# exosports/BART

Hardware: AMD Instinct MI355X
Metric: forward spectra/sec (100 layers x 1e4 wavenumbers) (higher is better)
Workload: dtype f64; 1 GPU; H2O+CO+CO2+CH4 eclipse, 100 layers x 10000 wavenumbers, 10 walkers batched per GPU per step (BASELINE config 3), opacity-table path, 27 T planes, H2-H2 CIA, 5 ray angles, toomuch 10, SURVEY 8d opacities, every step its own profile preparation; nlayers=100, nwave=10000, integ=1, cut=slant, cia_interp=spline, kappa_model=survey8d, parallelism=single GPU

## Files before the change

### bart_amd/build.py

```python
from __future__ import annotations

import os
import subprocess
import sys
from concurrent.futures import ThreadPoolExecutor

HERE = os.path.dirname(os.path.abspath(__file__))
CSRC = os.path.join(HERE, "csrc")
LIB = os.path.join(HERE, "libbartrt.so")
CLI = os.path.join(HERE, "transit")
SOURCES = ["rt_eclipse_angles.hip", "rt_eclipse_slant_ilp.hip", "rt_eclipse_qadj.hip", "rt_eclipse_i0.hip", "rt_eclipse_i1.hip", "rt_eclipse_i2.hip", "rt_eclipse_i0_ilp.hip", "rt_eclipse_i1_ilp.hip", "lbl.hip",
           "transit_geom.hip", "contrib.hip",
           "kernels.hip", "capi.hip", "engine.hip", "step.hip", "comm.hip", "mcmc.hip", "share.hip", "svc.hip", "rtc.hip", "io.cpp"]
HEADERS = ["engine.hpp", "kernels.hpp", "rt_eclipse.hpp", "rt_eclipse_s1.hpp", "rt_eclipse_s1s.hpp", "rt_eclipse_qadj.hpp", "kernel_table.inc", "imw_tab.hpp", "integ.hpp", "step.hpp", "lbl.hpp", "voigt_coef.hpp", "expint_coef.hpp", "prep.hpp", "io.hpp", "share.hpp", "svc.hpp", "svc_core.hpp", "rtc.hpp", "contrib.hpp", "comm.hpp", "devbuf.hpp",
           "transit_main.cpp", "../../include/bartrt.h"]


ILP = ["-mllvm", "-amdgpu-sched-strategy=max-ilp"]
EXTRA_FLAGS = {"rt_eclipse_i0_ilp.hip": ILP, "rt_eclipse_i1_ilp.hip": ILP, "rt_eclipse_slant_ilp.hip": ILP}
ANGLE_SIZES = tuple(int(x) for x in os.environ.get("BARTRT_AOT_ANGLES", "").split())
VARIANTS = {"rt_eclipse_angles.hip": [("rt_eclipse_a%d" % n, ["-DBARTRT_ANGLES=%d" % n, *ILP]) for n in ANGLE_SIZES]}
ANGLE_FLAG = "-DBARTRT_ANGLE_SIZES(X)=" + " ".join("X(%d)" % n for n in ANGLE_SIZES)

RT_OBJECT_PREFIXES = ("rt_eclipse_", "kernels", "engine")
BUILD_ID_INC = os.path.join(CSRC, "build_id.inc")


def _elf_section(blob: bytes, want: str):
    import struct
    if blob[:4] != b"\x7fELF" or blob[4] != 2:
        return None
    shoff, = struct.unpack_from("<Q", blob, 0x28)
    shentsize, shnum, shstrndx = struct.unpack_from("<HHH", blob, 0x3A)
    if shnum == 0:
# ... 146 lines not shown
```

### bart_amd/csrc/capi.hip

```cpp
#include <cstring>
#include <stdexcept>
#include <string>

#include "../../include/bartrt.h"
#include "comm.hpp"
#include "contrib.hpp"
#include "engine.hpp"
#include "lbl.hpp"
#include "share.hpp"
#include "step.hpp"
#include "rtc.hpp"
#include "svc.hpp"

#include <climits>
#include <cstdio>
#include <cstdlib>

#include <sys/stat.h>
#include <unistd.h>

using namespace bartrt;

static Engine *g_eng = nullptr;
static ChainService *g_svc = nullptr;
// ... 637 lines not shown
    if (ncolumns) *ncolumns = nc;
    if (wn_per_column) *wn_per_column = e->walked_info.wn_per_column;
    if (kernel && kernel_len > 0) {
      std::snprintf(kernel, (size_t)kernel_len, "%s%s%s%s", e->walked_info.kernel, e->walked_info.rtc ? " [instantiated at run time]" : "",
                    e->walked_info.prep_folded ? " [prepares its own walkers]" : "",
                    e->walked_info.window ? " [table through a moving window]" : "");
    }
    if (walked && n > 0) {
      if ((size_t)cap < (size_t)n * nc) throw std::invalid_argument("walked_end: buffer too small");
      HIPCHK(hipMemcpy(walked, e->d_walked, sizeof(int) * (size_t)n * nc, hipMemcpyDeviceToHost));
    }
    return BARTRT_OK;
  });
}

int bartrt_get_rtc_stats(int *available, int *compiled, int *from_disk, int *failed, double *compile_seconds) {
  const RtcStats st = rtc_stats();
  if (available) *available = rtc_available() ? 1 : 0;
  if (compiled) *compiled = st.compiled;
  if (from_disk) *from_disk = st.from_disk;
  if (failed) *failed = st.failed;
  if (compile_seconds) *compile_seconds = st.compile_seconds;
  return BARTRT_OK;
}

int bartrt_rtc_compile(const char *expr, int ilp, long *code_bytes) {
  if (!expr) return fail(BARTRT_EINVAL, "rtc_compile: null expression");
  std::string why;
  const long n = rtc_compile_only(expr, ilp != 0, why);
  if (code_bytes) *code_bytes = n;
// ... 278 lines not shown
```

### bart_amd/csrc/engine.hip

```cpp
#include "engine.hpp"
#include "lbl.hpp"
#include "contrib.hpp"
#include "share.hpp"
#include "step.hpp"
#include "svc.hpp"

#include <algorithm>
#include <climits>
#include <cmath>
#include <cstdlib>
#include <cstring>

#include <sys/stat.h>
#include <unistd.h>

namespace bartrt {

EngineStream::~EngineStream() {
  for (auto e : ev) (void)hipEventDestroy(e);
  if (stream) (void)hipStreamDestroy(stream);
}

Engine::~Engine() {
  delete step;
// ... 628 lines not shown
  pa.cloud_rup = cloud_rup; pa.cloud_rdown = cloud_rdown; pa.cloud_ext = cloud_ext;
  pa.coef = records.coef; pa.idx = records.idx; pa.kstop = records.kstop;
  pa.ok = d_okp ? d_okp : rec[0].ok.get();
  pa.rad_out = d_rad;
  pa.over = prep_over_once;
  pa.rtop = solution == 1 ? d_rtop.get() : nullptr;
  pa.ds = solution == 1 ? d_ds.get() : nullptr;
  return pa;
}

static int rt_block() {
  static const int b = [] { const char *e = std::getenv("BARTRT_BLOCK"); return e ? std::atoi(e) : 64; }();
  return (b == 128 || b == 256) ? b : 64;
}

RtArgs Engine::rt_args(const PrepArgs &pa, const Prefetch &pf, double *d_spec_out, bool want_tau, const double *d_ext,
                       bool lbl_fused, bool over_cloud, bool timed, hipStream_t st) {
  const int n = pa.nwalkers, block = rt_block();
  RtArgs r = rt;
  r.nwalkers = n;
  r.nsel = sel_walkers > n ? sel_walkers : 0;
  if (kernel_by_local) r.Wfull = r.W;
  r.coef = pa.coef; r.idx = pa.idx; r.kstop = pa.kstop;
  r.ext = d_ext;
  r.nprep = 0;
  if (pf.want_next) {
    const RecordSet &next = rec[1 - pf.bset];
    PrepArgs pn = pa;
    pn.nwalkers = pf_req_n;
    pn.prof = pf_req_prof;
// ... 15 lines not shown
  r.intens_out = nullptr;
  if (want_intens && n == 1 && solution == 0) {
    d_intens.reserve((size_t)A * W());
    r.intens_out = d_intens;
  }
  r.ntiles = (r.W + block - 1) / block;
  r.rtop = d_rtop; r.ds = d_ds;
  r.slog = nullptr;
  if (cut_slant && integ == 1 && solution == 0 && !lbl_fused) {
    const size_t need = slant_log_bytes(n, r.ntiles, block, A);
    if (need > d_slog.count()) {
      HIPCHK(hipDeviceSynchronize());
      d_slog.reserve(need);
    }
    r.slog = d_slog.get();
  }
  r.inv_starrad2 = solution == 1 ? 1.0 / (starrad * starrad) : 0.0;
  r.transparent = transparent ? 1 : 0;
  r.ev_start = r.ev_stop = nullptr;
  if (timed) {
    while ((int)ev.size() < ev_used + 2) {
      hipEvent_t e;
      HIPCHK(hipEventCreate(&e));
      ev.push_back(e);
    }
    if (lbl_fused) HIPCHK(hipEventRecord(ev[ev_used], st));
    else { r.ev_start = ev[ev_used]; r.ev_stop = ev[ev_used + 1]; }
  }
  r.walked_out = nullptr;
  if (want_walked && solution == 0 && !lbl_fused) {
// ... 61 lines not shown
```

### bart_amd/csrc/engine.hpp

```cpp
#pragma once
#include <hip/hip_runtime.h>

#include <string>
#include <vector>

#include "devbuf.hpp"
#include "io.hpp"
#include "kernels.hpp"

namespace bartrt {

hipError_t launch_prep(const PrepArgs &a, hipStream_t st);
hipError_t launch_rt(const RtArgs &a, int block, hipStream_t st, RtLaunchInfo *info = nullptr);
hipError_t launch_rt_folded(const RtArgs &a, const PrepArgs &prep, int block, hipStream_t st, RtLaunchInfo *info, bool *folded);
hipError_t launch_transit(const RtArgs &a, hipStream_t st, RtLaunchInfo *info = nullptr);
hipError_t launch_chord_table(const PrepArgs &a, hipStream_t st);
hipError_t launch_grid_transpose(const double *src, double *dst, long planes, int M, int W, hipStream_t st);

int parse_integ(const std::string &v);
int resolve_share_mode(const TCfg &cfg, bool no_service);

struct TableShare;
struct StepArgs;
struct Lbl;
// ... 83 lines not shown
  const double *pf_have_prof = nullptr;
  int pf_have_n = 0, pf_have_buf = 0;
  struct PrepSettings {
    double refradius, gsurf, cloudtop, scat_value, cloud_rup, cloud_rdown, cloud_ext;
    int has_cloud, scat_flag;
    bool operator==(const PrepSettings &o) const {
      return refradius == o.refradius && gsurf == o.gsurf && cloudtop == o.cloudtop && scat_value == o.scat_value &&
             cloud_rup == o.cloud_rup && cloud_rdown == o.cloud_rdown && cloud_ext == o.cloud_ext &&
             has_cloud == o.has_cloud && scat_flag == o.scat_flag;
    }
  };
  hipStream_t pf_have_stream = nullptr;
  PrepSettings pf_have_set{};
  int cap2 = 0;
  DevBuf<char> d_slog;
  StepArgs *step = nullptr;
  Lbl *lbl = nullptr;
  CfState *cf = nullptr;

  ~Engine();
  void init(int argc, const char **argv);
  void setup(const TCfg &cfg_in, int shard_rank, int shard_n);
  void read_settings();
  void generate_missing_opacity_file(int shard_rank);
  void read_atmosphere();
  void read_grid(OpacityHeader &oh, int shard_rank, int shard_n);
  void read_geometry();
  void open_device();
  void upload_table(const OpacityHeader &oh);
  void resample_cia(std::vector<double> &cia_planes, std::vector<double> &cia_temp);
// ... 24 lines not shown
```

### bart_amd/csrc/kernels.hip

```cpp
#include "integ.hpp"
#include "kernels.hpp"
#include "prep.hpp"

#include <cmath>
#include <cstdio>
#include <cstdlib>
#include <cstring>
#include <utility>

namespace bartrt {

template <int INTEG>
bool launch_rt_spec(const RtArgs &a, int block, hipStream_t st, KernelMode mode, bool force_window,
                    bool allow_sq, hipError_t &err, RtLaunchInfo *info, const PrepArgs *fold = nullptr);
extern template bool launch_rt_spec<0>(const RtArgs &, int, hipStream_t, KernelMode, bool, bool, hipError_t &, RtLaunchInfo *, const PrepArgs *);
extern template bool launch_rt_spec<1>(const RtArgs &, int, hipStream_t, KernelMode, bool, bool, hipError_t &, RtLaunchInfo *, const PrepArgs *);
extern template bool launch_rt_spec<2>(const RtArgs &, int, hipStream_t, KernelMode, bool, bool, hipError_t &, RtLaunchInfo *, const PrepArgs *);

__global__ __launch_bounds__(256) void prep_profiles(PrepArgs p) {
  extern __shared__ double sm[];
  prep_block(p, blockIdx.x, sm);
}

__device__ inline void block_to_work_g(int b, int nwalkers, int &tile, int &walker) {
// ... 169 lines not shown
    if (e != hipSuccess) return e;
    allowed = sh;
  }
  BARTRT_RT_LAUNCH((rt_eclipse<AT, -1, -1, INTEG>), dim3(nblocks), dim3(block), sh, st, a);
  return hipGetLastError();
}

KernelMode rt_kernel_mode() {
  static const KernelMode mode = [] {
    const char *e = std::getenv("BARTRT_KERNEL");
    if (!e || !*e) return KernelMode::kDefault;
    static const std::pair<const char *, KernelMode> names[] = {
        {"generic", KernelMode::kGeneric}, {"mono", KernelMode::kMono}, {"mono_occ", KernelMode::kMonoOcc},
        {"mono_ilp", KernelMode::kMonoIlp}, {"split", KernelMode::kSplit}, {"quad", KernelMode::kQuad},
        {"octo", KernelMode::kOcto}, {"hexa", KernelMode::kHexa}, {"r32", KernelMode::kR32},
        {"adj8", KernelMode::kAdj8}, {"adj16", KernelMode::kAdj16}};
    for (const auto &n : names)
      if (std::strcmp(e, n.first) == 0) return n.second;
    std::fprintf(stderr, "libbartrt: BARTRT_KERNEL=%s is not a kernel form (generic, mono, mono_occ, mono_ilp, split, quad, "
                         "octo, hexa, r32, adj8, adj16); ignored\n", e);
    return KernelMode::kDefault;
  }();
  return mode;
}
static bool rt_force_window() {
  static const bool v = std::getenv("BARTRT_WINDOW") != nullptr;
  return v;
}
static bool rt_allow_sq() {
  static const bool v = [] {
    const char *e = std::getenv("BARTRT_SQ");
    return !(e && e[0] == '0');
  }();
  return v;
}
// ... 43 lines not shown
```

### bart_amd/csrc/kernels.hpp

```cpp
#pragma once
#ifndef __HIPCC_RTC__
#include <hip/hip_runtime.h>
#include <hip/hip_ext.h>
#include <cstdint>
#else
typedef struct ihipEvent_t *hipEvent_t;
namespace std {
template <class T, T v> struct integral_constant { static constexpr T value = v; using value_type = T; constexpr operator T() const { return v; } };
using true_type = integral_constant<bool, true>;
using false_type = integral_constant<bool, false>;
template <bool B, class T, class F> struct conditional { using type = T; };
template <class T, class F> struct conditional<false, T, F> { using type = F; };
template <bool B, class T, class F> using conditional_t = typename conditional<B, T, F>::type;
}
#endif

#define BARTRT_MC_LIST(X) \
  X(1, 0) X(1, 1) X(1, 2) X(2, 0) X(2, 1) X(2, 2) X(3, 0) X(3, 1) X(3, 2) X(4, 0) X(4, 1) X(4, 2) \
  X(5, 0) X(5, 1) X(5, 2) X(6, 0) X(6, 1) X(6, 2)                                                 \
  X(1, 4) X(2, 4) X(3, 4) X(4, 4) X(5, 4) X(6, 4)
#define BARTRT_QADJ_LIST(X) BARTRT_MC_LIST(X)
#define BARTRT_EXT_C_LIST(X) X(0) X(1) X(2) X(4)

#define BARTRT_RT_LAUNCH(kernel, grid, block, sh, st, args) \
// ... 102 lines not shown
  int ref_ib;
  double ref_f;
  double ref_lnp;
  double gsurf, refradius;
  int scat_flag, iH2, iHe, has_cloud;
  double scat_value, cloudtop;
  double cloud_rup, cloud_rdown, cloud_ext;
  const double *over;
  double *coef;
  idx_t *idx;
  int *kstop;
  unsigned char *ok;
  double *rad_out;
  double *rtop;
  double *ds;
};

struct RtArgs {
  int L, M, Nt, C, A, W, nwalkers, ntiles;
  int nsel;
  int Wfull;
  const double *kappa;
  const double *cia;
  unsigned long long kappa_bytes, cia_bytes;
  int window;
  const double *ext;
  const double *wn;
  const double *coef;
  const idx_t *idx;
  const int *kstop;
// ... 2 lines not shown
  int cut_slant;
  double toomuch;
  double invmu[kMaxAngles];
  double wgt[kMaxAngles];
  double wq[kMaxAngles];
  double mu[kMaxAngles];
  double thr[kMaxAngles];
  double thrb[kMaxAngles];
  int drank[kMaxAngles];
  void *slog;
  double *spec;
  double *tau_out;
  int *last_out;
  double *intens_out;
  int *walked_out;
  const double *rtop, *ds;
  double inv_starrad2;
  int transparent;
  hipEvent_t ev_start, ev_stop;
  int nprep;
  PrepArgs prep_next;
};
__host__ __device__ inline int prep_slots(int nprep) { return (nprep + 7) / 8 * 8; }

inline void slant_thresholds(RtArgs &r) {
  for (int a = 0; a < r.A; a++) {
    const double im = r.invmu[a];
    double t = r.toomuch / im;
    if (!(t == t) || t > 1.7e308 || t < 0.0) { r.thr[a] = t < 0.0 ? -1.0 : 1.7976931348623157e308; continue; }
    for (int it = 0; it < 64 && t * im > r.toomuch; it++) t = __builtin_nextafter(t, 0.0);
// ... 15 lines not shown
inline size_t slant_log_bytes(int nwalkers, int ntiles, int block, int A) {
  return (size_t)nwalkers * (size_t)ntiles * (size_t)block * (size_t)A * 20u;
}

struct RtLaunchInfo {
  const char *kernel = "";
  int wn_per_column = 64;
  int ncolumns = 0;
  bool prep_fused = false;
  bool prep_folded = false;
  bool rtc = false;
  bool window = false;
};

#ifndef __HIPCC_RTC__
enum class KernelMode { kDefault, kGeneric, kMono, kMonoOcc, kMonoIlp, kSplit, kQuad, kOcto, kHexa, kR32, kAdj8, kAdj16 };
KernelMode rt_kernel_mode();
#endif

constexpr double kExpShift = 6755399441055744.0;
constexpr double kExpMin = -708.0;

__device__ __forceinline__ double exp_scale(double p, double shifted) {
  const int hi = __double2hiint(p) + (__double2loint(shifted) << 20);
  return __hiloint2double(hi, __double2loint(p));
}

__device__ __forceinline__ double exp_core(double x) {
  const double t = fma(x, 1.4426950408889634074, kExpShift);
  const double n = t - kExpShift;
  double r = fma(n, -6.93147180369123816490e-01, x);
// ... 146 lines not shown
```

### bart_amd/csrc/rt_eclipse.hpp

```cpp
#pragma once
#include "integ.hpp"
#include "kernels.hpp"
#include "prep.hpp"

#ifndef __HIPCC_RTC__
#include <cmath>
#include <cstdlib>
#include <type_traits>
#include <utility>
#endif

#ifndef BARTRT_WPE
#define BARTRT_WPE 4
#endif

namespace bartrt {

constexpr long kQuadMaxColumns = 640, kQuadMaxColumnsSimpson = 480;
constexpr long kQuadRaysMaxColumns = 80;
constexpr long kOctoRaysMaxColumns = 40;
constexpr int kFoldMaxWorkgroups = 512;
constexpr long kOctoMaxColumns = 400;
constexpr long kSplitMinColumns = 1025, kSplitMaxColumns = 1300;
constexpr long kIlpMaxColumns = 20000;
// ... 653 lines not shown
      };
      swap_angles(0, i);
      if (j == 0) j = i;
      swap_angles(r.A - 1, j);
      return true;
    }
  return false;
}

bool launch_rt_fast_ilp(const RtArgs &b, bool sq, int block, int nblocks, size_t sh, hipStream_t st, hipError_t &err);
bool launch_rt_fast_ext(const RtArgs &b, bool sq, int block, int nblocks, size_t sh, hipStream_t st, hipError_t &err);

bool launch_rt_slant(const RtArgs &b, int integ, bool sq, int block, int nblocks, size_t sh, hipStream_t st, hipError_t &err);
bool launch_rt_slant_ext(const RtArgs &b, int integ, bool sq, int block, int nblocks, size_t sh, hipStream_t st, hipError_t &err);
bool launch_rt_slant_out(const RtArgs &b, int block, int nblocks, size_t sh, hipStream_t st, hipError_t &err);

bool launch_rt_qadj(const RtArgs &b, bool sq, int rows, int nblocks, size_t sh, hipStream_t st, hipError_t &err);

#ifndef BARTRT_ANGLE_SIZES
#define BARTRT_ANGLE_SIZES(X)
#endif
#define BARTRT_DECL_ANGLES(N) \
  bool launch_rt_angles_##N(const RtArgs &b, int integ, int block, int nblocks, size_t sh, hipStream_t st, hipError_t &err);
BARTRT_ANGLE_SIZES(BARTRT_DECL_ANGLES)
#undef BARTRT_DECL_ANGLES

struct SpecLaunch {
  const RtArgs &a;
  RtArgs b;
  bool sq = false;
// ... 146 lines not shown
  static_assert(INTEG != kIntegSimpson, "the one-ray-per-lane form: rules 0 / 2");
  const LpGeom g = lp_geom(c, rows, 64 / rows / 5);
  const RtArgs &b = g.b;
  return (dispatch_mc(b.M, b.C, false, [&](auto m, auto cc, auto) {
            constexpr int M = decltype(m)::value, C = decltype(cc)::value;
            c.run(rows == 8 ? rt_eclipse_quad<5, M, C, false, 8, INTEG, true> : rt_eclipse_quad<5, M, C, false, 4, INTEG, true>,
                  g.nwg, 256, g.lds, b);
          }) ||
          rtc_try(c.info, false, dim3(g.nwg), dim3(256), g.lds, c.st, b, c.err, "rt_eclipse_quad<5, %d, %d, false, %d, %d, true>",
                  b.M, b.C, rows, INTEG)) &&
         c.launched(rows == 8 ? "rt_eclipse_quad<R=8, one ray per lane>" : "rt_eclipse_quad<R=4, one ray per lane>", g.wn, g.ncolumns,
                    false, b.window != 0);
}

template <int INTEG>
bool launch_form_slant(const SpecLaunch &c) {
  const RtArgs &b = c.b;
  const int nwg = c.workgroups(b.ntiles);
  const size_t lds = c.sh + c.shp;
  return (launch_rt_slant(b, INTEG, c.sq, c.block, nwg, lds, c.st, c.err) ||
          (rtc_single_wave_ok(b) &&
           (INTEG == kIntegSimpson
                ? rtc_try(c.info, true, dim3(nwg), dim3(c.block), lds, c.st, b, c.err, "rt_eclipse_simpson_slant<5, %d, %d, %s, %d>",
                          b.M, b.C, tf(c.sq), slant_sched(b.M, b.C, 1))
                : rtc_try(c.info, true, dim3(nwg), dim3(c.block), lds, c.st, b, c.err, "rt_eclipse_fast<5, %d, %d, %s, %d, 1, false, true>",
                          b.M, b.C, tf(c.sq), INTEG)))) &&
         c.launched(INTEG == kIntegSimpson ? "rt_eclipse_simpson_slant (ILP-scheduled build)" : "rt_eclipse_fast<SLANT> (ILP-scheduled build)",
                    c.block, b.ntiles);
}

template <int INTEG>
bool launch_form_quad(const SpecLaunch &c, int rows) {
  const LpGeom g = lp_geom(c, rows, 64 / rows);
  const RtArgs &b = g.b;
// ... 92 lines not shown
        const LpGeom g = lp_geom(c, adj_rows, 64 / adj_rows);
        if (fold && !g.folds) return false;
        if (launch_form_qadj(c, g, adj_rows)) return true;
      }
      const bool lp_forced = mode == KernelMode::kQuad || mode == KernelMode::kOcto || mode == KernelMode::kHexa ||
                             mode == KernelMode::kR32 || mode == KernelMode::kAdj8 || mode == KernelMode::kAdj16;
      if ((lp_forced || (dflt && other != kVarSingle)) && c.addressable(rows)) {
        const LpGeom g = lp_geom(c, rows, 64 / rows);
        if (fold && !g.folds) return false;
        if (launch_form_quad_allr<INTEG>(c, g, rows)) return true;
      }
      if (fold) return false;
    } else if ((mode == KernelMode::kQuad || mode == KernelMode::kOcto || (dflt && columns <= kQuadRaysMaxColumns)) && fits32) {
      if (launch_form_quad_rays<INTEG>(c, mode == KernelMode::kOcto || (dflt && columns <= kOctoRaysMaxColumns) ? 8 : 4)) return true;
    }
    return launch_form_slant<INTEG>(c);
  }
  constexpr long quad_max = INTEG == kIntegSimpson ? kQuadMaxColumnsSimpson : kQuadMaxColumns;
  if ((mode == KernelMode::kQuad || mode == KernelMode::kOcto || (dflt && columns <= quad_max)) && fits32 &&
      launch_form_quad<INTEG>(c, octo ? 8 : 4))
    return true;
  if constexpr (INTEG != kIntegSimpson) {
    if ((mode == KernelMode::kSplit || (dflt && columns >= kSplitMinColumns && columns <= kSplitMaxColumns)) &&
        launch_form_split<INTEG>(c))
      return true;
  }
  return launch_form_single<INTEG>(c, mode != KernelMode::kMonoOcc && (mode == KernelMode::kMonoIlp || columns < kIlpMaxColumns));
}

#endif
}
// ... 1 lines not shown
```

### bart_amd/csrc/rt_eclipse_s1s.hpp

```cpp
#pragma once
#include "integ.hpp"
#include "kernels.hpp"
#include "rt_eclipse_s1.hpp"

#ifndef __HIPCC_RTC__
#include <type_traits>
#endif

namespace bartrt {

#ifndef BARTRT_FLAG_CLAMP
#define BARTRT_FLAG_CLAMP 1
#endif
template <int A>
__device__ __forceinline__ double alive_flags(const RtArgs &p, double tm, double (&m)[A]) {
  double n = 0.0;
#if BARTRT_FLAG_CLAMP
  const double tb = tm * -4.149515568880993e180;
#pragma unroll
  for (int a = 0; a < A; a++) {
    asm("v_add_f64 %0, %1, %2 clamp" : "=v"(m[a]) : "v"(tb), "s"(p.thrb[a]));
    n += m[a];
  }
#else
#pragma unroll
  for (int a = 0; a < A; a++) {
    m[a] = tm <= p.thr[a] ? 1.0 : 0.0;
    n += m[a];
  }
#endif
  return n;
}

template <int AT, int MT, int CT, bool SQ, int SCHED = 1, bool EXT = false, bool OUT = false>
__global__ __launch_bounds__(256) __attribute__((amdgpu_waves_per_eu(OUT ? 1 : 2, BARTRT_WPE)))
void rt_eclipse_simpson_slant(RtArgs p) {
  extern __shared__ double smem[];
  constexpr int A = AT, M = MT, C = CT;
  constexpr int NC = 4 + 2 * M + 2 * C, NI = 1 + C, NLD = 2 * M + 2 * C;
  constexpr int NR = NLD + (EXT ? 1 : 0) > 0 ? NLD + (EXT ? 1 : 0) : 1;
  constexpr int AE = SQ ? A - 1 : A;
  constexpr int kBlk = 6;
  static_assert(kBlk - 2 <= kSimpsonPad, "the radius table's overrun entries");
  const int L = p.L, W = p.W;
  int bid = blockIdx.x;
  if (p.nprep > 0) {
    if (bid < p.nprep) { prep_block(p.prep_next, bid, smem); return; }
    bid -= prep_slots(p.nprep);
    if (bid < 0) return;
  }
  int tile, w;
  block_to_work(bid, p.nwalkers, tile, w);
  if (tile >= p.ntiles) return;

  double *sC = smem;
  idx_t *sI = reinterpret_cast<idx_t *>(smem + (size_t)L * NC);
  double *sWw = smem + (size_t)L * NC + (size_t)L * NI;
  const double *sW = sWw;
  stage2_to_lds(sC, p.coef + (size_t)w * L * NC, L * NC, sI, p.idx + (size_t)w * L * NI, L * NI, threadIdx.x,
                blockDim.x);
  const int kraw = p.kstop[w], kend = kstop_layer(kraw);
  const bool deck_on = kstop_deck(kraw);
  __syncthreads();
  simpson_radius_table(sWw, sC, NC, L, kend, threadIdx.x, blockDim.x);
  __syncthreads();

  const int i = tile * blockDim.x + threadIdx.x;
  const bool valid = i < W;
  const unsigned ii = valid ? (unsigned)i : (unsigned)(W - 1);
  const double nu = p.wn[ii];
  const double bnum = 2.0 * kH * nu * nu * nu * kLS * kLS;
  const double nu4 = (nu * nu) * (nu * nu);
  const TableLoader<M, C> tab(p, ii, sI);
  const double *extw = EXT ? p.ext + (size_t)w * L * W + ii : nullptr;
  auto load_layer = [&](int k, double (&r)[NR]) {
    tab.load(k, r);
    if constexpr (EXT) r[NLD] = extw[(size_t)(L - 1 - k) * W];
  };
  const double tcap = tau_cap(p, A);
  const int kcut = kend < L - 2 ? kend : L - 2;
  double thr_max = p.thr[0];
#pragma unroll
  for (int a = 1; a < A; a++) thr_max = p.thr[a] > thr_max ? p.thr[a] : thr_max;

  double s_even = 0.0, eprev = 0.0, e2 = 0.0;
  double x1 = 0.0, h0 = 0.0, r0 = 1.0, tm = 0.0;
  [[maybe_unused]] int out_last = 0;
  [[maybe_unused]] double out_tau = 0.0;
  double y1[A], y2[A], P0[A], P1[A];
#pragma unroll
  for (int a = 0; a < A; a++) { y1[a] = y2[a] = P0[a] = P1[a] = 0.0; }
  const unsigned nth = blockDim.x;
  const unsigned lsh = (unsigned)__builtin_ctz(nth) + 4u;
  const unsigned log_bytes = nth * (unsigned)A * 20u;
  const auto rs_log = __builtin_amdgcn_make_buffer_rsrc(
      reinterpret_cast<char *>(p.slog) + ((size_t)w * p.ntiles + tile) * log_bytes, 0, (int)log_bytes, 0x00020000);
  const unsigned log_k0 = nth * (unsigned)A * 16u + threadIdx.x * 4u;
#pragma unroll
  for (int sl = 0; sl < A; sl++) __builtin_amdgcn_raw_buffer_store_b32(-1, rs_log, (int)(log_k0 + sl * nth * 4u), 0, 0);
  double nprev = (double)A;
  const unsigned tid16 = threadIdx.x * 16u;
  auto log_event = [&](double nnow, int kev) {
    const bool ev = nnow < nprev;
    const unsigned slot = (unsigned)((double)A - nprev);
    const unsigned off = ev ? (slot << lsh) + tid16 : 0x7ffffff0u;
    const unsigned offk = ev ? log_k0 + (slot << (lsh - 2u)) : 0x7ffffff0u;
    v4u_t v;
    v.x = (unsigned)__double2loint(x1); v.y = (unsigned)__double2hiint(x1);
    v.z = (unsigned)__double2loint(h0); v.w = (unsigned)__double2hiint(h0);
    __builtin_amdgcn_raw_buffer_store_b128(v, rs_log, (int)off, 0, 0);
    __builtin_amdgcn_raw_buffer_store_b32(kev, rs_log, (int)offk, 0, 0);
    nprev = nnow;
  };

  auto layer = [&](auto Jc, auto Fc, auto Mc, int k0, const double (&r)[NR], const double (&cf)[NC],
// ... 92 lines not shown
    constexpr bool MASKED = decltype(Mc)::value;
    auto inblk = [&](int k) { return MASKED ? clampk(k) : k; };
    layer(integral_constant<int, 0>{}, Fc, Mc, k0, s0, cfE, cfO);
    load_layer(inblk(k0 + 3), s0);
    layer(integral_constant<int, 1>{}, Fc, Mc, k0, s1, cfO, cfE);
    load_layer(inblk(k0 + 4), s1);
    layer(integral_constant<int, 2>{}, Fc, Mc, k0, s2, cfE, cfO);
    load_layer(inblk(k0 + 5), s2);
    layer(integral_constant<int, 3>{}, Fc, Mc, k0, s0, cfO, cfE);
    load_layer(clampk(k0 + 6), s0);
    layer(integral_constant<int, 4>{}, Fc, Mc, k0, s1, cfE, cfO);
    load_layer(clampk(k0 + 7), s1);
    layer(integral_constant<int, 5>{}, Fc, Mc, k0, s2, cfO, cfE);
    load_layer(clampk(k0 + 8), s2);
  };
  load_layer(clampk(0), s0);
  load_layer(clampk(1), s1);
  load_layer(clampk(2), s2);
  if constexpr (SCHED != 0) {
#pragma unroll
    for (int j = 0; j < NC; j++) cfE[j] = sC[j];
  }
  auto any_active = [&]() {
    unsigned long long mk = __ballot(tm <= thr_max);
    asm volatile("" : "+s"(mk));
    return mk != 0ull;
  };
  int kw = kBlk;
  if (kcut >= kBlk - 1) {
    block6(true_type{}, false_type{}, 0);
    int k0 = kBlk;
    bool alive = any_active();
    if (alive & (k0 + kBlk - 1 <= kcut)) {
      do {
        block6(false_type{}, false_type{}, k0);
        k0 += kBlk;
        alive = any_active();
      } while (alive & (k0 + kBlk - 1 <= kcut));
    }
    kw = k0;
    if (alive & (k0 <= kend)) {
      block6(false_type{}, true_type{}, k0);
      kw = k0 + kBlk;
    }
// ... 113 lines not shown
      if constexpr (OUT) {
        if (p.intens_out && valid && !fast_ok) p.intens_out[(size_t)a * W + i] = Ia;
      }
    }
    F = fast_ok ? F_fast : F;
  }
  if constexpr (OUT) {
    if (p.tau_out && valid) {
      for (int kk = out_last + 1; kk < L; kk++) p.tau_out[(size_t)i * L + kk] = out_tau;
      p.last_out[i] = out_last;
    }
  }
  if (valid) p.spec[(size_t)w * W + i] = F;
  if (p.walked_out && threadIdx.x == 0)
    p.walked_out[(size_t)w * p.ntiles + tile] = (kw < kend + 1 ? kw : kend + 1);
}


}
```

### include/bartrt.h

```cpp
#ifndef BARTRT_H
#define BARTRT_H

#ifdef __cplusplus
extern "C" {
#endif

#define BARTRT_OK        0
#define BARTRT_EINVAL   -1
#define BARTRT_EIO      -2
#define BARTRT_ENODEV   -3
#define BARTRT_ENOTSUP  -4


int bartrt_init(int argc, const char **argv);

int bartrt_get_no_samples(void);

int bartrt_get_waveno_arr(double *out, int n);

int bartrt_set_radius(double refradius_km);

int bartrt_set_cloudtop(double log10_pbar);

int bartrt_set_scattering(int flag, double value);
// ... 99 lines not shown
                     double *band, double *full, int *status);
int bartrt_cf_params_dev(const double *d_params, int nwalkers, int npars, int kind,
                         double *d_band, double *d_full, int *d_status, void *stream);

int bartrt_get_lbl_extinction(const double *prof, int nprof, double *ext,
                              int nlayers, int nwave);

int bartrt_voigt(const double *x, const double *y, double *k, long n);

int bartrt_timing_begin(void);
int bartrt_timing_begin_sampled(int stride);
int bartrt_timing_end(double *kernel_ms, int *nlaunch);
int bartrt_walked_begin(void);
int bartrt_walked_end(int *walked, int cap, int *nwalkers, int *ncolumns, int *wn_per_column,
                      char *kernel, int kernel_len);
int bartrt_get_rtc_stats(int *available, int *compiled, int *from_disk, int *failed, double *compile_seconds);
int bartrt_rtc_compile(const char *expr, int ilp, long *code_bytes);
double bartrt_algorithmic_bytes(int nwalkers);

#ifdef __cplusplus
}
#endif
#endif
```

Baseline: 95230 spectra/s.

## Split slant-path columns across waves with task lists and cross-wave state handoff

Adds a task-list form of the Simpson slant kernel for 5 angles and one-wave blocks. A host-built schedule spreads each walker's columns over a fixed number of waves per walker, about one per SIMD. A column can be cut at a 6-layer boundary: the wave holding its first part saves its integration state to global memory and publishes a ready flag. The wave holding the rest polls that flag and resumes, or recomputes the column from the top on its own log if the flag does not arrive in time. The aim is to balance layer work across SIMDs and remove the tail where some SIMDs get two columns and others one, at the cost of extra state traffic, spin-polling and possible duplicate work.

```diff
diff --git a/bart_amd/build.py b/bart_amd/build.py
--- a/bart_amd/build.py
+++ b/bart_amd/build.py
@@ -9,15 +9,15 @@
 CSRC = os.path.join(HERE, "csrc")
 LIB = os.path.join(HERE, "libbartrt.so")
 CLI = os.path.join(HERE, "transit")
-SOURCES = ["rt_eclipse_angles.hip", "rt_eclipse_slant_ilp.hip", "rt_eclipse_qadj.hip", "rt_eclipse_i0.hip", "rt_eclipse_i1.hip", "rt_eclipse_i2.hip", "rt_eclipse_i0_ilp.hip", "rt_eclipse_i1_ilp.hip", "lbl.hip",
+SOURCES = ["rt_eclipse_angles.hip", "rt_eclipse_slant_ilp.hip", "rt_eclipse_slant_tasks.hip", "rt_eclipse_qadj.hip", "rt_eclipse_i0.hip", "rt_eclipse_i1.hip", "rt_eclipse_i2.hip", "rt_eclipse_i0_ilp.hip", "rt_eclipse_i1_ilp.hip", "lbl.hip",
            "transit_geom.hip", "contrib.hip",
            "kernels.hip", "capi.hip", "engine.hip", "step.hip", "comm.hip", "mcmc.hip", "share.hip", "svc.hip", "rtc.hip", "io.cpp"]
-HEADERS = ["engine.hpp", "kernels.hpp", "rt_eclipse.hpp", "rt_eclipse_s1.hpp", "rt_eclipse_s1s.hpp", "rt_eclipse_qadj.hpp", "kernel_table.inc", "imw_tab.hpp", "integ.hpp", "step.hpp", "lbl.hpp", "voigt_coef.hpp", "expint_coef.hpp", "prep.hpp", "io.hpp", "share.hpp", "svc.hpp", "svc_core.hpp", "rtc.hpp", "contrib.hpp", "comm.hpp", "devbuf.hpp",
+HEADERS = ["engine.hpp", "kernels.hpp", "rt_eclipse.hpp", "rt_eclipse_s1.hpp", "rt_eclipse_s1s.hpp", "rt_eclipse_qadj.hpp", "kernel_table.inc", "imw_tab.hpp", "integ.hpp", "step.hpp", "lbl.hpp", "voigt_coef.hpp", "expint_coef.hpp", "prep.hpp", "io.hpp", "share.hpp", "svc.hpp", "svc_core.hpp", "rtc.hpp", "contrib.hpp", "comm.hpp", "devbuf.hpp", "split_sched.hpp",
            "transit_main.cpp", "../../include/bartrt.h"]
 
 
 ILP = ["-mllvm", "-amdgpu-sched-strategy=max-ilp"]
-EXTRA_FLAGS = {"rt_eclipse_i0_ilp.hip": ILP, "rt_eclipse_i1_ilp.hip": ILP, "rt_eclipse_slant_ilp.hip": ILP}
+EXTRA_FLAGS = {"rt_eclipse_i0_ilp.hip": ILP, "rt_eclipse_i1_ilp.hip": ILP, "rt_eclipse_slant_ilp.hip": ILP, "rt_eclipse_slant_tasks.hip": ILP}
 ANGLE_SIZES = tuple(int(x) for x in os.environ.get("BARTRT_AOT_ANGLES", "").split())
 VARIANTS = {"rt_eclipse_angles.hip": [("rt_eclipse_a%d" % n, ["-DBARTRT_ANGLES=%d" % n, *ILP]) for n in ANGLE_SIZES]}
 ANGLE_FLAG = "-DBARTRT_ANGLE_SIZES(X)=" + " ".join("X(%d)" % n for n in ANGLE_SIZES)
diff --git a/bart_amd/csrc/capi.hip b/bart_amd/csrc/capi.hip
--- a/bart_amd/csrc/capi.hip
+++ b/bart_amd/csrc/capi.hip
@@ -6,6 +6,7 @@
 #include "comm.hpp"
 #include "contrib.hpp"
 #include "engine.hpp"
+#include "split_sched.hpp"
 #include "lbl.hpp"
 #include "share.hpp"
 #include "step.hpp"
@@ -675,6 +676,23 @@
   });
 }
 
+int bartrt_split_schedule(int nwalkers, int ntiles, int nlayers, int simds, int *waves, int waves_cap, int *tasks,
+                          int tasks_cap, int *nwaves, int *ntasks, long *max_layers, long *plain_layers, int *pays) {
+  SplitSched sc;
+  const bool any = split_schedule(nwalkers, ntiles, nlayers, simds, sc);
+  if (nwaves) *nwaves = any ? sc.nwaves : 0;
+  if (ntasks) *ntasks = any ? (int)(sc.tasks.size() / kSplitTaskInts) : 0;
+  if (max_layers) *max_layers = sc.max_layers;
+  if (plain_layers) *plain_layers = sc.plain_layers;
+  if (pays) *pays = any && split_pays(sc) ? 1 : 0;
+  if (!any) return BARTRT_OK;
+  if ((waves && (size_t)waves_cap < sc.waves.size()) || (tasks && (size_t)tasks_cap < sc.tasks.size()))
+    return fail(BARTRT_EINVAL, "split_schedule: buffer too small");
+  if (waves) std::copy(sc.waves.begin(), sc.waves.end(), waves);
+  if (tasks) std::copy(sc.tasks.begin(), sc.tasks.end(), tasks);
+  return BARTRT_OK;
+}
+
 int bartrt_get_rtc_stats(int *available, int *compiled, int *from_disk, int *failed, double *compile_seconds) {
   const RtcStats st = rtc_stats();
   if (available) *available = rtc_available() ? 1 : 0;
diff --git a/bart_amd/csrc/engine.hip b/bart_amd/csrc/engine.hip
--- a/bart_amd/csrc/engine.hip
+++ b/bart_amd/csrc/engine.hip
@@ -1,4 +1,5 @@
 #include "engine.hpp"
+#include "split_sched.hpp"
 #include "lbl.hpp"
 #include "contrib.hpp"
 #include "share.hpp"
@@ -666,6 +667,45 @@
   return (b == 128 || b == 256) ? b : 64;
 }
 
+void Engine::split_args(RtArgs &r) {
+  r.split = SplitArgs{};
+  if (split_simds == 0) {
+    hipDeviceProp_t prop;
+    HIPCHK(hipGetDeviceProperties(&prop, device));
+    split_simds = prop.multiProcessorCount * 4;
+    if (const char *e = std::getenv("BARTRT_SPLIT_SIMDS")) { const int v = std::atoi(e); if (v > 0 && v < split_simds) split_simds = v; }
+    if (const char *e = std::getenv("BARTRT_SPLIT_POLLS")) split_polls = std::max(0, std::atoi(e));
+  }
+  const SplitPlan *plan = nullptr;
+  for (const SplitPlan &sp : split_plans)
+    if (sp.nwalkers == r.nwalkers && sp.ntiles == r.ntiles && sp.L == r.L) { plan = &sp; break; }
+  if (!plan) {
+    SplitSched sc;
+    SplitPlan sp{r.nwalkers, r.ntiles, r.L, false, false, 0, {}, {}};
+    sp.any = split_schedule(r.nwalkers, r.ntiles, r.L, split_simds, sc);
+    if (sp.any) {
+      sp.pays = split_pays(sc);
+      sp.nwaves = sc.nwaves;
+      sp.waves.upload(sc.waves);
+      sp.tasks.upload(sc.tasks);
+      if (!d_split_state.get()) {
+        d_split_state.reserve((size_t)split_simds * (8 + 4 * 5) * 64);
+        d_split_ready.reserve((size_t)split_simds);
+        d_split_log.reserve((size_t)split_simds * slant_log_bytes(1, 1, 64, 5));
+        HIPCHK(hipMemset(d_split_ready, 0, (size_t)split_simds * sizeof(unsigned long long)));
+      }
+    }
+    split_plans.push_back(std::move(sp));
+    plan = &split_plans.back();
+  }
+  if (!plan->any) return;
+  if (++split_serial == 0) split_serial = 1;
+  r.split.waves = plan->waves; r.split.tasks = plan->tasks;
+  r.split.state = d_split_state; r.split.ready = d_split_ready; r.split.altlog = d_split_log;
+  r.split.serial = split_serial; r.split.polls = split_polls;
+  r.split.nwaves = plan->nwaves; r.split.pays = plan->pays ? 1 : 0;
+}
+
 RtArgs Engine::rt_args(const PrepArgs &pa, const Prefetch &pf, double *d_spec_out, bool want_tau, const double *d_ext,
                        bool lbl_fused, bool over_cloud, bool timed, hipStream_t st) {
   const int n = pa.nwalkers, block = rt_block();
@@ -711,6 +751,7 @@
       d_slog.reserve(need);
     }
     r.slog = d_slog.get();
+    if (A == 5 && block == 64 && r.nprep == 0 && !d_ext && !r.tau_out && !r.intens_out) split_args(r);
   }
   r.inv_starrad2 = solution == 1 ? 1.0 / (starrad * starrad) : 0.0;
   r.transparent = transparent ? 1 : 0;
diff --git a/bart_amd/csrc/engine.hpp b/bart_amd/csrc/engine.hpp
--- a/bart_amd/csrc/engine.hpp
+++ b/bart_amd/csrc/engine.hpp
@@ -121,6 +121,20 @@
   PrepSettings pf_have_set{};
   int cap2 = 0;
   DevBuf<char> d_slog;
+  struct SplitPlan {
+    int nwalkers, ntiles, L;
+    bool any, pays;
+    int nwaves;
+    DevBuf<int> waves, tasks;
+  };
+  std::vector<SplitPlan> split_plans;
+  DevBuf<double> d_split_state;
+  DevBuf<unsigned long long> d_split_ready;
+  DevBuf<char> d_split_log;
+  unsigned split_serial = 0;
+  int split_simds = 0;
+  int split_polls = 64;
+  void split_args(RtArgs &r);
   StepArgs *step = nullptr;
   Lbl *lbl = nullptr;
   CfState *cf = nullptr;
diff --git a/bart_amd/csrc/kernels.hip b/bart_amd/csrc/kernels.hip
--- a/bart_amd/csrc/kernels.hip
+++ b/bart_amd/csrc/kernels.hip
@@ -207,11 +207,12 @@
         {"generic", KernelMode::kGeneric}, {"mono", KernelMode::kMono}, {"mono_occ", KernelMode::kMonoOcc},
         {"mono_ilp", KernelMode::kMonoIlp}, {"split", KernelMode::kSplit}, {"quad", KernelMode::kQuad},
         {"octo", KernelMode::kOcto}, {"hexa", KernelMode::kHexa}, {"r32", KernelMode::kR32},
-        {"adj8", KernelMode::kAdj8}, {"adj16", KernelMode::kAdj16}};
+        {"adj8", KernelMode::kAdj8}, {"adj16", KernelMode::kAdj16},
+        {"mono_tasks", KernelMode::kMonoTasks}, {"mono_plain", KernelMode::kMonoPlain}};
     for (const auto &n : names)
       if (std::strcmp(e, n.first) == 0) return n.second;
     std::fprintf(stderr, "libbartrt: BARTRT_KERNEL=%s is not a kernel form (generic, mono, mono_occ, mono_ilp, split, quad, "
-                         "octo, hexa, r32, adj8, adj16); ignored\n", e);
+                         "octo, hexa, r32, adj8, adj16, mono_tasks, mono_plain); ignored\n", e);
     return KernelMode::kDefault;
   }();
   return mode;
diff --git a/bart_amd/csrc/kernels.hpp b/bart_amd/csrc/kernels.hpp
--- a/bart_amd/csrc/kernels.hpp
+++ b/bart_amd/csrc/kernels.hpp
@@ -140,6 +140,20 @@
   double *rad_out;
   double *rtop;
   double *ds;
+};
+
+constexpr int kSplitTaskInts = 4;
+constexpr int kSplitToEnd = 0x7fffffff;
+struct SplitArgs {
+  const int *waves;
+  const int *tasks;
+  double *state;
+  unsigned long long *ready;
+  char *altlog;
+  unsigned serial;
+  int polls;
+  int nwaves;
+  int pays;
 };
 
 struct RtArgs {
@@ -172,6 +186,7 @@
   int *last_out;
   double *intens_out;
   int *walked_out;
+  SplitArgs split;
   const double *rtop, *ds;
   double inv_starrad2;
   int transparent;
@@ -217,7 +232,8 @@
 };
 
 #ifndef __HIPCC_RTC__
-enum class KernelMode { kDefault, kGeneric, kMono, kMonoOcc, kMonoIlp, kSplit, kQuad, kOcto, kHexa, kR32, kAdj8, kAdj16 };
+enum class KernelMode { kDefault, kGeneric, kMono, kMonoOcc, kMonoIlp, kSplit, kQuad, kOcto, kHexa, kR32, kAdj8, kAdj16,
+                        kMonoTasks, kMonoPlain };
 KernelMode rt_kernel_mode();
 #endif
 
diff --git a/bart_amd/csrc/rt_eclipse.hpp b/bart_amd/csrc/rt_eclipse.hpp
--- a/bart_amd/csrc/rt_eclipse.hpp
+++ b/bart_amd/csrc/rt_eclipse.hpp
@@ -691,6 +691,7 @@
 bool launch_rt_slant(const RtArgs &b, int integ, bool sq, int block, int nblocks, size_t sh, hipStream_t st, hipError_t &err);
 bool launch_rt_slant_ext(const RtArgs &b, int integ, bool sq, int block, int nblocks, size_t sh, hipStream_t st, hipError_t &err);
 bool launch_rt_slant_out(const RtArgs &b, int block, int nblocks, size_t sh, hipStream_t st, hipError_t &err);
+bool launch_rt_slant_tasks(const RtArgs &b, bool sq, size_t sh, hipStream_t st, hipError_t &err);
 
 bool launch_rt_qadj(const RtArgs &b, bool sq, int rows, int nblocks, size_t sh, hipStream_t st, hipError_t &err);
 
@@ -867,10 +868,16 @@
 }
 
 template <int INTEG>
-bool launch_form_slant(const SpecLaunch &c) {
+bool launch_form_slant(const SpecLaunch &c, KernelMode mode) {
   const RtArgs &b = c.b;
   const int nwg = c.workgroups(b.ntiles);
   const size_t lds = c.sh + c.shp;
+  if constexpr (INTEG == kIntegSimpson) {
+    const bool tasks = b.split.waves && b.nprep == 0 && c.block == 64 && mode != KernelMode::kMonoPlain &&
+                       (b.split.pays || mode == KernelMode::kMonoTasks);
+    if (tasks && launch_rt_slant_tasks(b, c.sq, c.sh, c.st, c.err))
+      return c.launched("rt_eclipse_simpson_slant (ILP-scheduled build) [split columns]", c.block, b.ntiles);
+  }
   return (launch_rt_slant(b, INTEG, c.sq, c.block, nwg, lds, c.st, c.err) ||
           (rtc_single_wave_ok(b) &&
            (INTEG == kIntegSimpson
@@ -993,7 +1000,7 @@
     } else if ((mode == KernelMode::kQuad || mode == KernelMode::kOcto || (dflt && columns <= kQuadRaysMaxColumns)) && fits32) {
       if (launch_form_quad_rays<INTEG>(c, mode == KernelMode::kOcto || (dflt && columns <= kOctoRaysMaxColumns) ? 8 : 4)) return true;
     }
-    return launch_form_slant<INTEG>(c);
+    return launch_form_slant<INTEG>(c, mode);
   }
   constexpr long quad_max = INTEG == kIntegSimpson ? kQuadMaxColumnsSimpson : kQuadMaxColumns;
   if ((mode == KernelMode::kQuad || mode == KernelMode::kOcto || (dflt && columns <= quad_max)) && fits32 &&
diff --git a/bart_amd/csrc/rt_eclipse_s1s.hpp b/bart_amd/csrc/rt_eclipse_s1s.hpp
--- a/bart_amd/csrc/rt_eclipse_s1s.hpp
+++ b/bart_amd/csrc/rt_eclipse_s1s.hpp
@@ -32,8 +32,8 @@
   return n;
 }
 
-template <int AT, int MT, int CT, bool SQ, int SCHED = 1, bool EXT = false, bool OUT = false>
-__global__ __launch_bounds__(256) __attribute__((amdgpu_waves_per_eu(OUT ? 1 : 2, BARTRT_WPE)))
+template <int AT, int MT, int CT, bool SQ, int SCHED = 1, bool EXT = false, bool OUT = false, bool TASKS = false>
+__global__ __launch_bounds__(256) __attribute__((amdgpu_waves_per_eu((OUT || TASKS) ? 1 : 2, BARTRT_WPE)))
 void rt_eclipse_simpson_slant(RtArgs p) {
   extern __shared__ double smem[];
   constexpr int A = AT, M = MT, C = CT;
@@ -42,16 +42,26 @@
   constexpr int AE = SQ ? A - 1 : A;
   constexpr int kBlk = 6;
   static_assert(kBlk - 2 <= kSimpsonPad, "the radius table's overrun entries");
+  static_assert(!TASKS || (!EXT && !OUT), "the task-list form: the plain table path");
   const int L = p.L, W = p.W;
   int bid = blockIdx.x;
-  if (p.nprep > 0) {
-    if (bid < p.nprep) { prep_block(p.prep_next, bid, smem); return; }
-    bid -= prep_slots(p.nprep);
-    if (bid < 0) return;
-  }
   int tile, w;
-  block_to_work(bid, p.nwalkers, tile, w);
-  if (tile >= p.ntiles) return;
+  [[maybe_unused]] int t_cur = 0, t_end = 0;
+  if constexpr (TASKS) {
+    t_cur = p.split.waves[2 * bid];
+    w = p.split.waves[2 * bid + 1];
+    t_end = p.split.waves[2 * bid + 2];
+    if (t_cur >= t_end) return;
+    tile = 0;
+  } else {
+    if (p.nprep > 0) {
+      if (bid < p.nprep) { prep_block(p.prep_next, bid, smem); return; }
+      bid -= prep_slots(p.nprep);
+      if (bid < 0) return;
+    }
+    block_to_work(bid, p.nwalkers, tile, w);
+    if (tile >= p.ntiles) return;
+  }
 
   double *sC = smem;
   idx_t *sI = reinterpret_cast<idx_t *>(smem + (size_t)L * NC);
@@ -64,6 +74,32 @@
   __syncthreads();
   simpson_radius_table(sWw, sC, NC, L, kend, threadIdx.x, blockDim.x);
   __syncthreads();
+
+  do {
+  [[maybe_unused]] int klim = kSplitToEnd, slot = 0, k_from = 0;
+  [[maybe_unused]] bool fresh = true, own_log = false;
+  if constexpr (TASKS) {
+    const int *tk = p.split.tasks + (size_t)t_cur * kSplitTaskInts;
+    tile = tk[0];
+    klim = tk[2];
+    slot = tk[3];
+    if (tk[1] > 0) {
+      unsigned long long *rw = p.split.ready + slot;
+      own_log = true;
+      for (int n = 0; n < p.split.polls; n++) {
+        const unsigned long long v = __hip_atomic_load(rw, __ATOMIC_RELAXED, __HIP_MEMORY_SCOPE_AGENT);
+        const unsigned hi = (unsigned)__builtin_amdgcn_readfirstlane((int)(unsigned)(v >> 32));
+        if (hi == p.split.serial) {
+          k_from = __builtin_amdgcn_readfirstlane((int)(unsigned)v);
+          fresh = false;
+          own_log = false;
+          break;
+        }
+        __builtin_amdgcn_s_sleep(16);
+      }
+      if (!fresh) __builtin_amdgcn_fence(__ATOMIC_ACQUIRE, "agent");
+    }
+  }
 
   const int i = tile * blockDim.x + threadIdx.x;
   const bool valid = i < W;
@@ -93,12 +129,31 @@
   const unsigned nth = blockDim.x;
   const unsigned lsh = (unsigned)__builtin_ctz(nth) + 4u;
   const unsigned log_bytes = nth * (unsigned)A * 20u;
-  const auto rs_log = __builtin_amdgcn_make_buffer_rsrc(
-      reinterpret_cast<char *>(p.slog) + ((size_t)w * p.ntiles + tile) * log_bytes, 0, (int)log_bytes, 0x00020000);
+  char *logp = reinterpret_cast<char *>(p.slog) + ((size_t)w * p.ntiles + tile) * log_bytes;
+  if constexpr (TASKS) {
+    if (own_log) logp = p.split.altlog + (size_t)blockIdx.x * log_bytes;
+  }
+  const auto rs_log = __builtin_amdgcn_make_buffer_rsrc(logp, 0, (int)log_bytes, 0x00020000);
   const unsigned log_k0 = nth * (unsigned)A * 16u + threadIdx.x * 4u;
-#pragma unroll
-  for (int sl = 0; sl < A; sl++) __builtin_amdgcn_raw_buffer_store_b32(-1, rs_log, (int)(log_k0 + sl * nth * 4u), 0, 0);
+  if (!TASKS || fresh) {
+#pragma unroll
+    for (int sl = 0; sl < A; sl++) __builtin_amdgcn_raw_buffer_store_b32(-1, rs_log, (int)(log_k0 + sl * nth * 4u), 0, 0);
+  }
   double nprev = (double)A;
+  [[maybe_unused]] double *const st_lane =
+      TASKS ? p.split.state + (size_t)slot * ((8 + 4 * A) * 64) + threadIdx.x : nullptr;
+  if constexpr (TASKS) {
+    if (!fresh) {
+      const double *st = st_lane;
+      s_even = st[0 * 64]; eprev = st[1 * 64]; e2 = st[2 * 64]; x1 = st[3 * 64];
+      h0 = st[4 * 64]; r0 = st[5 * 64]; tm = st[6 * 64]; nprev = st[7 * 64];
+#pragma unroll
+      for (int a = 0; a < A; a++) {
+        y1[a] = st[(8 + a) * 64]; y2[a] = st[(8 + A + a) * 64];
+        P0[a] = st[(8 + 2 * A + a) * 64]; P1[a] = st[(8 + 3 * A + a) * 64];
+      }
+    }
+  }
   const unsigned tid16 = threadIdx.x * 16u;
   auto log_event = [&](double nnow, int kev) {
     const bool ev = nnow < nprev;
@@ -221,12 +276,12 @@
     layer(integral_constant<int, 5>{}, Fc, Mc, k0, s2, cfO, cfE);
     load_layer(clampk(k0 + 8), s2);
   };
-  load_layer(clampk(0), s0);
-  load_layer(clampk(1), s1);
-  load_layer(clampk(2), s2);
+  load_layer(clampk(k_from), s0);
+  load_layer(clampk(k_from + 1), s1);
+  load_layer(clampk(k_from + 2), s2);
   if constexpr (SCHED != 0) {
 #pragma unroll
-    for (int j = 0; j < NC; j++) cfE[j] = sC[j];
+    for (int j = 0; j < NC; j++) cfE[j] = sC[(TASKS ? clampk(k_from) * NC : 0) + j];
   }
   auto any_active = [&]() {
     unsigned long long mk = __ballot(tm <= thr_max);
@@ -234,7 +289,42 @@
     return mk != 0ull;
   };
   int kw = kBlk;
-  if (kcut >= kBlk - 1) {
+  if constexpr (TASKS) {
+    int k0 = k_from;
+    if (fresh) {
+      if (kcut >= kBlk - 1) block6(true_type{}, false_type{}, 0);
+      else block6(true_type{}, true_type{}, 0);
+      k0 = kBlk;
+    }
+    bool alive = any_active();
+    while (alive & (k0 + kBlk - 1 <= kcut) & (k0 < klim)) {
+      block6(false_type{}, false_type{}, k0);
+      k0 += kBlk;
+      alive = any_active();
+    }
+    if (klim != kSplitToEnd) {
+      double *st = st_lane;
+      st[0 * 64] = s_even; st[1 * 64] = eprev; st[2 * 64] = e2; st[3 * 64] = x1;
+      st[4 * 64] = h0; st[5 * 64] = r0; st[6 * 64] = tm; st[7 * 64] = nprev;
+#pragma unroll
+      for (int a = 0; a < A; a++) {
+        st[(8 + a) * 64] = y1[a]; st[(8 + A + a) * 64] = y2[a];
+        st[(8 + 2 * A + a) * 64] = P0[a]; st[(8 + 3 * A + a) * 64] = P1[a];
+      }
+      asm volatile("s_waitcnt vmcnt(0)" ::: "memory");
+      __builtin_amdgcn_fence(__ATOMIC_RELEASE, "agent");
+      asm volatile("s_waitcnt vmcnt(0)" ::: "memory");
+      if (threadIdx.x == 0)
+        __hip_atomic_store(p.split.ready + slot, ((unsigned long long)p.split.serial << 32) | (unsigned)k0,
+                           __ATOMIC_RELAXED, __HIP_MEMORY_SCOPE_AGENT);
+      continue;
+    }
+    kw = k0;
+    if (alive & (k0 <= kend)) {
+      block6(false_type{}, true_type{}, k0);
+      kw = k0 + kBlk;
+    }
+  } else if (kcut >= kBlk - 1) {
     block6(true_type{}, false_type{}, 0);
     int k0 = kBlk;
     bool alive = any_active();
@@ -378,6 +468,7 @@
   if (valid) p.spec[(size_t)w * W + i] = F;
   if (p.walked_out && threadIdx.x == 0)
     p.walked_out[(size_t)w * p.ntiles + tile] = (kw < kend + 1 ? kw : kend + 1);
+  } while (TASKS && ++t_cur < t_end);
 }
 
 
diff --git a/bart_amd/csrc/rt_eclipse_slant_tasks.hip b/bart_amd/csrc/rt_eclipse_slant_tasks.hip
--- /dev/null
+++ b/bart_amd/csrc/rt_eclipse_slant_tasks.hip
@@ -0,0 +1,24 @@
+#include "rt_eclipse.hpp"
+
+#ifndef BARTRT_SLANT_SCHED
+#define BARTRT_SLANT_SCHED 1
+#endif
+
+namespace bartrt {
+
+bool launch_rt_slant_tasks(const RtArgs &b, bool sq, size_t sh, hipStream_t st, hipError_t &err) {
+#define BARTRT_SLANT_TASKS(MM, CC)                                                                                       \
+  if (b.M == MM && b.C == CC) {                                                                                          \
+    if (sq) BARTRT_RT_LAUNCH((rt_eclipse_simpson_slant<5, MM, CC, true, slant_sched(MM, CC, BARTRT_SLANT_SCHED), false, false, true>), \
+                             dim3(b.split.nwaves), dim3(64), sh, st, b);                                                 \
+    else BARTRT_RT_LAUNCH((rt_eclipse_simpson_slant<5, MM, CC, false, slant_sched(MM, CC, BARTRT_SLANT_SCHED), false, false, true>),   \
+                          dim3(b.split.nwaves), dim3(64), sh, st, b);                                                    \
+    err = hipGetLastError();                                                                                             \
+    return true;                                                                                                         \
+  }
+  BARTRT_MC_LIST(BARTRT_SLANT_TASKS)
+#undef BARTRT_SLANT_TASKS
+  return false;
+}
+
+}
diff --git a/bart_amd/csrc/split_sched.hpp b/bart_amd/csrc/split_sched.hpp
--- /dev/null
+++ b/bart_amd/csrc/split_sched.hpp
@@ -0,0 +1,73 @@
+#pragma once
+#include <algorithm>
+#include <vector>
+
+#include "kernels.hpp"
+
+namespace bartrt {
+
+constexpr int kSplitBlk = 6;
+
+struct SplitSched {
+  std::vector<int> waves;
+  std::vector<int> tasks;
+  int nwaves = 0;
+  int nsplit = 0;
+  long max_layers = 0;
+  long plain_layers = 0;
+};
+
+inline bool split_schedule(int nwalkers, int ntiles, int L, int simds, SplitSched &s) {
+  s = SplitSched{};
+  if (nwalkers <= 0 || ntiles <= 0 || L <= 0 || simds <= 0) return false;
+  const long columns = (long)nwalkers * ntiles;
+  s.plain_layers = (columns + simds - 1) / simds * L;
+  const int wpw = simds / nwalkers;
+  if (wpw < 1 || wpw >= ntiles) return false;
+  const long total = (long)ntiles * L;
+  const int last_cut = (L - 1) / kSplitBlk * kSplitBlk;
+  std::vector<long> cut(wpw + 1, 0);
+  for (int j = 1; j < wpw; j++) {
+    const long x = (total * j + wpw / 2) / wpw;
+    const long col = x / L;
+    long off = (x % L + kSplitBlk / 2) / kSplitBlk * kSplitBlk;
+    if (off > last_cut) off = (x % L) * 2 >= (long)last_cut + L ? L : last_cut;
+    cut[j] = std::max(cut[j - 1], col * L + off);
+  }
+  cut[wpw] = total;
+  std::vector<int> wave_j, wave_w;
+  for (int g = 0; g * 8 < wpw; g++)
+    for (int w = 0; w < nwalkers; w++)
+      for (int x = 0; x < 8 && g * 8 + x < wpw; x++) { wave_j.push_back(g * 8 + x); wave_w.push_back(w); }
+  s.nwaves = (int)wave_j.size();
+  std::vector<std::vector<int>> block_of(nwalkers, std::vector<int>(wpw, 0));
+  for (int b = 0; b < s.nwaves; b++) block_of[wave_w[b]][wave_j[b]] = b;
+  auto push = [&](int tile, int kb, int ke, int slot) {
+    s.tasks.push_back(tile); s.tasks.push_back(kb); s.tasks.push_back(ke); s.tasks.push_back(slot);
+  };
+  for (int b = 0; b < s.nwaves; b++) {
+    const int j = wave_j[b], w = wave_w[b];
+    s.waves.push_back((int)(s.tasks.size() / kSplitTaskInts));
+    s.waves.push_back(w);
+    const long lo = cut[j], hi = cut[j + 1];
+    s.max_layers = std::max(s.max_layers, hi - lo);
+    if (hi <= lo) continue;
+    const int c_lo = (int)(lo / L), k_lo = (int)(lo % L);
+    const int c_hi = (int)(hi / L), k_hi = (int)(hi % L);
+    if (k_hi > 0) push(c_hi, 0, k_hi, b);
+    for (int c = c_lo + (k_lo > 0 ? 1 : 0); c < c_hi; c++) push(c, 0, kSplitToEnd, 0);
+    if (k_lo > 0) push(c_lo, k_lo, kSplitToEnd, block_of[w][j - 1]);
+    if (k_lo > 0 && w == 0) s.nsplit++;
+  }
+  s.nsplit *= nwalkers;
+  s.waves.push_back((int)(s.tasks.size() / kSplitTaskInts));
+  s.waves.push_back(0);
+  return s.nsplit > 0;
+}
+
+constexpr double kSplitPaysBelow = 0.90;
+inline bool split_pays(const SplitSched &s) {
+  return s.nsplit > 0 && (double)(s.max_layers + kSplitBlk) <= kSplitPaysBelow * (double)s.plain_layers;
+}
+
+}
diff --git a/include/bartrt.h b/include/bartrt.h
--- a/include/bartrt.h
+++ b/include/bartrt.h
@@ -137,6 +137,8 @@
 int bartrt_walked_begin(void);
 int bartrt_walked_end(int *walked, int cap, int *nwalkers, int *ncolumns, int *wn_per_column,
                       char *kernel, int kernel_len);
+int bartrt_split_schedule(int nwalkers, int ntiles, int nlayers, int simds, int *waves, int waves_cap, int *tasks,
+                          int tasks_cap, int *nwaves, int *ntasks, long *max_layers, long *plain_layers, int *pays);
 int bartrt_get_rtc_stats(int *available, int *compiled, int *from_disk, int *failed, double *compile_seconds);
 int bartrt_rtc_compile(const char *expr, int ilp, long *code_bytes);
 double bartrt_algorithmic_bytes(int nwalkers);
```

Result: slower. 63870 spectra/s (-32.9%).
